# Axe--/Visual-Question-Answering

Measured on AMD Instinct MI355X. Metric: QA-pairs/sec (train step, attention model, K=1000), higher is better.
Workload: dtype f32

## Files before the change

include/coattn.h:

```cpp
#ifndef COATTN_H
#define COATTN_H

#include <stddef.h>
#include <stdint.h>

#ifdef __cplusplus
extern "C" {
#endif

#define COATTN_F32 0
#define COATTN_BF16 1

#define COATTN_IMPL_AUTO 0
#define COATTN_IMPL_GENERAL 1
#define COATTN_IMPL_FUSED 2
#define COATTN_FLAG_BF16_PROJ 4
#define COATTN_FLAG_BF16_IN 8
#define COATTN_FLAG_EXACT3 16
#define COATTN_FLAG_SPLIT2 32
#define COATTN_FLAG_F16PAIR 64
#define COATTN_FLAG_FAST16 128
#define COATTN_FLAG_BILINEAR 256
typedef struct coattn_params {
  const void* W_v; const void* b_v;
// ... 178 lines not shown
int coattn_bn_exact_geometry(int B, int H, int W, int C, int dtype, int* out);
size_t coattn_bn_exact_workspace_bytes(int B, int H, int W, int C);
int coattn_bn_exact_forward(const void* x, const void* gamma, const void* beta, void* running_mean, void* running_var,
                            double momentum, double eps, void* y, void* save_mean, void* save_invstd, void* ws, int B, int H,
                            int W, int C, int pool, int relu, int dtype, void* stream);

int coattn_conv1_bn_exact_supported(int B, int H, int W, int Cin, int Cout, int pool, int dtype);
size_t coattn_conv1_bn_exact_workspace_bytes(int B, int H, int W, int with_x);
int coattn_conv1_bn_exact_forward(const void* image, const void* weight, const void* gamma, const void* beta, void* running_mean,
                                  void* running_var, double momentum, double eps, void* x_out, void* y, void* save_mean,
                                  void* save_invstd, void* ws, int B, int H, int W, int Cin, int Cout, int pool, int dtype,
                                  void* stream);
int coattn_conv1_probe(const void* image, const void* weight, void* x, void* ws, int B, int H, int W, int order, int step,
                       int halves, int skip, void* stream);

typedef struct coattn_lstm_params      { const void *w_ih, *w_hh, *b_ih, *b_hh; } coattn_lstm_params;
typedef struct coattn_lstm_param_grads { void *w_ih, *w_hh, *b_ih, *b_hh; } coattn_lstm_param_grads;
int coattn_lstm_supported(int B, int T, int E, int H, int dtype);
int coattn_lstm_workspace_bytes(int B, int T, int E, int H, int dtype, size_t* saved, size_t* ws_fwd, size_t* ws_bwd);
int coattn_lstm_forward(const void* X, const int32_t* len, const coattn_lstm_params* p, void* out, void* x_masked,
                        void* saved, void* ws, int B, int T, int E, int H, int dtype, int flags, void* stream);
int coattn_lstm_backward(const void* X, const int32_t* len, const coattn_lstm_params* p, const void* out, const void* saved,
                         const void* g_out, const void* g_xmasked, void* dX, const coattn_lstm_param_grads* pg,
                         int accumulate, void* ws, int B, int T, int E, int H, int dtype, int flags, void* stream);

#define COATTN_IDS_I32 0
#define COATTN_IDS_I64 1
#define COATTN_EMBEDDING_CHUNK 32
int coattn_embedding_supported(long long n, long long V, int E, int dtype);
int coattn_embedding_workspace_bytes(long long n, long long V, int E, int dtype, size_t* ws_bwd);
// ... 70 lines not shown
```

visual-question-answering_amd/_lib.py:

```python
from __future__ import annotations

import ctypes as C
import os
import subprocess

_HERE = os.path.dirname(os.path.abspath(__file__))
LIB_PATH = os.environ.get("COATTN_LIB_PATH") or os.path.join(_HERE, "libcoattn_hip.so")
CSRC = os.path.join(_HERE, "csrc")

EXPORTS = ("coattn_version", "coattn_last_error", "coattn_fused_supported", "coattn_workspace_bytes",
           "coattn_forward", "coattn_attention_forward", "coattn_backward", "coattn_gemm_f32", "coattn_gemm_bf16",
           "coattn_phrase_workspace_bytes", "coattn_phrase_forward", "coattn_phrase_backward",
           "coattn_ce_workspace_bytes", "coattn_ce_forward", "coattn_linear_workspace_bytes", "coattn_linear_forward",
           "coattn_linear_wgrad_workspace_bytes", "coattn_linear_weight_grad",
           "coattn_head_workspace_bytes", "coattn_head_forward", "coattn_head_backward", "coattn_head_status",
           "coattn_ce_status", "coattn_p2p_enable_peer", "coattn_p2p_reduce_scatter", "coattn_p2p_all_gather",
           "coattn_profile_begin", "coattn_profile_end", "coattn_features_native", "coattn_status",
           "coattn_phrase_status", "coattn_status_accumulate", "coattn_phrase_status_accumulate", "coattn_infer",
           "coattn_forward_len", "coattn_infer_len", "coattn_attention_forward_len", "coattn_backward_len",
           "coattn_forward_maps", "coattn_forward_maps_len", "coattn_backward_maps", "coattn_backward_maps_len",
           "coattn_alt_workspace_bytes", "coattn_alt_forward", "coattn_alt_backward",
           "coattn_soft_loss_forward", "coattn_vqa_score", "coattn_head_forward_soft",
           "coattn_adam_workspace_bytes", "coattn_adam_step",
           "coattn_bn_supported", "coattn_bn_workspace_bytes", "coattn_bn_relu_pool_forward", "coattn_relu_pool_forward",
           "coattn_bn_exact_geometry", "coattn_bn_exact_workspace_bytes", "coattn_bn_exact_forward",
           "coattn_conv1_bn_exact_supported", "coattn_conv1_bn_exact_workspace_bytes", "coattn_conv1_bn_exact_forward",
           "coattn_conv1_probe",
           "coattn_lstm_supported", "coattn_lstm_workspace_bytes", "coattn_lstm_forward", "coattn_lstm_backward",
           "coattn_embedding_supported", "coattn_embedding_workspace_bytes", "coattn_embedding_forward",
           "coattn_embedding_backward",
           "coattn_dropout_supported", "coattn_dropout_forward", "coattn_dropout_backward",
           "coattn_features_gather_supported", "coattn_features_gather",
           "coattn_overlay_supported", "coattn_overlay_render")

F32 = 0
IDS_I32, IDS_I64 = 0, 1
BF16 = 1
IMPL_AUTO, IMPL_GENERAL, IMPL_FUSED = 0, 1, 2
FLAG_BF16_PROJ = 4
FLAG_BF16_IN = 8
FLAG_EXACT3 = 16
FLAG_SPLIT2 = 32
# ... 123 lines not shown
                                  + _int("accumulate dtype flags") + _void("stream")),
}
DROPOUT_SIGNATURES = {
    "coattn_dropout_forward": (_void("x0 y0 x1 y1") + _i64("n") + _of(C.c_float)("p") + _void("state") + _int("advance")
                               + _void("stream")),
    "coattn_dropout_backward": _void("g dx") + _i64("n") + _of(C.c_float)("p") + _void("state stream"),
}
FEATURES_SIGNATURES = {
    "coattn_features_gather": (_void("table") + _int("table_dtype") + _void("idx") + _int("idx_dtype") + _void("out bad_idx")
                               + _i64("S B") + _int("N d flags") + _void("stream")),
}
OVERLAY_SIGNATURES = {
    "coattn_overlay_render": (_void("image") + _i64("sB sC sH sW") + _void("a_v a_q q_len") + (("p", C.POINTER(OverlayParams)),)
                              + _void("out bad_maps") + _int("B L H W Gh Gw T strip_h mode") + _void("stream")),
}
_TABLE = {**SIGNATURES, **EMBEDDING_SIGNATURES, **DROPOUT_SIGNATURES, **FEATURES_SIGNATURES, **OVERLAY_SIGNATURES}
_INDEX = {name: {n: i for i, (n, _) in enumerate(sig)} for name, sig in _TABLE.items()}
_DEFAULTS = dict.fromkeys("q_len av_out aq_out saved g_av g_aq dV labels loss g_loss g_logits dv dq bad_ids bad_idx x1 y1 bad_maps".split())
_DEFAULTS.update(dv_sB=0, dv_sN=0, dv_sD=0)


def ptr(t):
    return C.c_void_p(t.data_ptr()) if t is not None else C.c_void_p(0)


def ptr_array(tensors):
    return (C.c_void_p * len(tensors))(*[t.data_ptr() for t in tensors])


def rows(t):
    step = t.stride(0) * t.element_size()
# ... 126 lines not shown
    lib.coattn_bn_workspace_bytes.restype = C.c_size_t
    lib.coattn_bn_relu_pool_forward.argtypes = ([C.c_void_p] * 6 + [C.c_double] * 2 + [C.c_void_p] * 3 + [C.c_int] * 7
                                                + [C.c_void_p])
    lib.coattn_relu_pool_forward.argtypes = [C.c_void_p] * 2 + [C.c_int] * 5 + [C.c_void_p]
    lib.coattn_bn_exact_geometry.argtypes = [C.c_int] * 5 + [C.POINTER(C.c_int)]
    lib.coattn_bn_exact_workspace_bytes.argtypes = [C.c_int] * 4
    lib.coattn_bn_exact_workspace_bytes.restype = C.c_size_t
    lib.coattn_bn_exact_forward.argtypes = ([C.c_void_p] * 5 + [C.c_double] * 2 + [C.c_void_p] * 4 + [C.c_int] * 7
                                            + [C.c_void_p])
    lib.coattn_conv1_bn_exact_supported.argtypes = [C.c_int] * 7
    lib.coattn_conv1_bn_exact_workspace_bytes.argtypes = [C.c_int] * 4
    lib.coattn_conv1_bn_exact_workspace_bytes.restype = C.c_size_t
    lib.coattn_conv1_bn_exact_forward.argtypes = ([C.c_void_p] * 6 + [C.c_double] * 2 + [C.c_void_p] * 5 + [C.c_int] * 7
                                                  + [C.c_void_p])
    lib.coattn_conv1_probe.argtypes = [C.c_void_p] * 4 + [C.c_int] * 7 + [C.c_void_p]
    lib.coattn_lstm_supported.argtypes = [C.c_int] * 5
    lib.coattn_lstm_workspace_bytes.argtypes = [C.c_int] * 5 + [C.POINTER(C.c_size_t)] * 3
    lib.coattn_lstm_forward.argtypes = ([C.c_void_p] * 2 + [C.POINTER(LstmParams)] + [C.c_void_p] * 4 + [C.c_int] * 6
                                        + [C.c_void_p])
    lib.coattn_lstm_backward.argtypes = ([C.c_void_p] * 2 + [C.POINTER(LstmParams)] + [C.c_void_p] * 5
                                         + [C.POINTER(LstmParamGrads)] + [C.c_int] + [C.c_void_p] + [C.c_int] * 6
                                         + [C.c_void_p])
    lib.coattn_embedding_supported.argtypes = [C.c_int64, C.c_int64, C.c_int, C.c_int]
    lib.coattn_embedding_workspace_bytes.argtypes = [C.c_int64, C.c_int64, C.c_int, C.c_int, C.POINTER(C.c_size_t)]
    lib.coattn_dropout_supported.argtypes = [C.c_int64]
    lib.coattn_features_gather_supported.argtypes = [C.c_int64, C.c_int64, C.c_int, C.c_int, C.c_int, C.c_int]
    lib.coattn_overlay_supported.argtypes = [C.c_int] * 9
    _lib = lib
    return lib

# ... 137 lines not shown
```

visual-question-answering_amd/csrc/api.hip:

```cpp
#include "common.h"
#include "fused.h"

#include <string.h>

static thread_local char g_err[512] = "";

void coattn_set_error(const char* fmt, ...) {
  va_list ap;
  va_start(ap, fmt);
  vsnprintf(g_err, sizeof(g_err), fmt, ap);
  va_end(ap);
}

extern "C" int coattn_version(void) { return 2100; }

namespace {
constexpr int kProfMax = 48;
struct Prof {
  bool on = false;
  int n = 0, created = 0;
  hipEvent_t ev[kProfMax + 1];
  const char* name[kProfMax];
};
thread_local Prof g_prof;
}

void prof_mark(hipStream_t s, const char* name) {
  Prof& p = g_prof;
  if (!p.on || p.n >= kProfMax) return;
// ... 837 lines not shown
```

visual-question-answering_amd/csrc/encoder.hip:

```cpp
#include <math.h>

#include "common.h"

namespace {

constexpr int kThreads = 256;
constexpr int kMaxStatBlocks = 2048;
constexpr int kPixelsPerStatBlock = 400;
constexpr int kMaxNormBlocks = 4096;
constexpr int kStatLoads = 8;

typedef double f64x2 __attribute__((ext_vector_type(2)));

inline int stat_blocks(int64_t pixels) {
  const int64_t g = pixels / kPixelsPerStatBlock;
  return g < 1 ? 1 : g > kMaxStatBlocks ? kMaxStatBlocks : (int)g;
}

inline size_t partial_bytes(int G, int C) { return (size_t)G * C * sizeof(f64x2); }

__global__ __launch_bounds__(kThreads) void bn_stats_partial_kernel(const f32x4* __restrict__ x, f64x2* __restrict__ partial,
                                                                    int64_t total4, int c4) {
  __shared__ double sh[8][kThreads];
  const int tid = threadIdx.x;
// ... 181 lines not shown
  }
  running_mean[xg] = nm;
  running_var[xg] = nv;
  save_mean[xg] = mean;
  save_invstd[xg] = invstd;
}

constexpr int kConv1Terms = 32;
constexpr int kConv1Mfmas = kConv1Terms / 2;
constexpr int kConv1Pixels = 32;

template <int D>
__device__ __forceinline__ constexpr int conv1_term(int i, int g) { return (i / D) * 2 * D + g * D + i % D; }

template <int D>
__global__ __launch_bounds__(128) void conv1_stats_miopen_kernel(
    const float* __restrict__ image, const float* __restrict__ weight, float* __restrict__ x, float* __restrict__ partial, int B,
    int H, int W, int g1, int ngrps) {
  __shared__ float lds[kConv1Pixels * 64 * 2];
  const int hh = threadIdx.x >> 6, lane = threadIdx.x & 63, g = lane >> 5, p = lane & 31;
  const int HW = H * W;
  const int pbase = blockIdx.x * kConv1Pixels, pix = pbase + p;
  const bool live = pix < HW;
  const bool full = pbase + kConv1Pixels <= HW;
  const int h = pix / W, w = pix - h * W;
  const int ch = 32 * hh + p;
  float wt[kConv1Mfmas];
  int off[kConv1Mfmas];
  unsigned real = 0;
#pragma unroll
  for (int i = 0; i < kConv1Mfmas; ++i) {
    const int k = conv1_term<D>(i, g);
    const int tap = k / 3, c = k - 3 * tap, ky = tap / 3, kx = tap - 3 * ky;
    const int ih = h + ky - 1, iw = w + kx - 1;
    const bool in = live && k < 27 && ih >= 0 && ih < H && iw >= 0 && iw < W;
    off[i] = in ? (ih * W + iw) * 3 + c : 0;
    real |= in ? 1u << i : 0u;
    const float wk = weight[ch * 27 + (k < 27 ? k : 26)];
    wt[i] = k < 27 ? wk : 0.f;
  }
  const int64_t sample = (int64_t)HW * 3;
  float even[kConv1Mfmas], odd[kConv1Mfmas];
  const float* image1 = image + (B > 1 ? sample : 0);
#pragma unroll
  for (int i = 0; i < kConv1Mfmas; ++i) even[i] = image[off[i]];
#pragma unroll
  for (int i = 0; i < kConv1Mfmas; ++i) odd[i] = image1[off[i]];
  float sum[16], sq[16];
#pragma unroll
  for (int v = 0; v < 16; ++v) sum[v] = sq[v] = 0.f;
  float* xo = x + ((int64_t)(pbase + 4 * g) * 64 + ch);
  const int64_t xstep = (int64_t)HW * 64;
  auto one_sample = [&](float (&terms)[kConv1Mfmas], int n) {
    const float* ahead = image + (int64_t)(n + 2 < B ? n + 2 : B - 1) * sample;
    f32x16 acc;
#pragma unroll
    for (int e = 0; e < 16; ++e) acc[e] = 0.f;
#pragma unroll
    for (int i = 0; i < kConv1Mfmas; ++i) {
      const float t = (real >> i) & 1u ? terms[i] : 0.f;
      acc = __builtin_amdgcn_mfma_f32_32x32x2f32(t, wt[i], acc, 0, 0, 0);
      terms[i] = ahead[off[i]];
    }
    if (full) {
#pragma unroll
      for (int v = 0; v < 16; ++v) {
        xo[(8 * (v >> 2) + (v & 3)) * 64] = acc[v];
        sum[v] += acc[v];
        sq[v] = __builtin_fmaf(acc[v], acc[v], sq[v]);
      }
    } else {
#pragma unroll
      for (int v = 0; v < 16; ++v)
        if (pbase + 8 * (v >> 2) + 4 * g + (v & 3) < HW) {
          xo[(8 * (v >> 2) + (v & 3)) * 64] = acc[v];
          sum[v] += acc[v];
          sq[v] = __builtin_fmaf(acc[v], acc[v], sq[v]);
        }
    }
    xo += xstep;
  };
  for (int n = 0; n < B; n += 2) {
    one_sample(even, n);
    if (n + 1 < B) one_sample(odd, n + 1);
  }
#pragma unroll
  for (int v = 0; v < 16; ++v) {
    const int o = ((8 * (v >> 2) + 4 * g + (v & 3)) * 64 + ch) * 2;
    lds[o] = sum[v];
    lds[o + 1] = sq[v];
  }
  __syncthreads();
  for (int red = g1 >> 1; red > 0; red >>= 1) {
#pragma unroll
    for (int v = 0; v < 16; ++v) {
// ... 62 lines not shown
    if (step == 0) {
      sacc = __builtin_fmaf(a, v, sacc);
    } else {
      const float prod = __fmul_rn(a, v);
      sacc = __fadd_rn(prod, sacc);
    }
  }
  x[i] = halves == 2 ? __fadd_rn(acc[0], acc[1]) : acc[0];
}

struct Affine {
  float mean[4], lo[4], scale[4], beta[4], gamma[4];
};

template <bool STOCK>
__device__ __forceinline__ f32x4 affine(const f32x4 v, const Affine& a) {
  f32x4 t;
#pragma unroll
  for (int e = 0; e < 4; ++e)
    t[e] = STOCK ? __builtin_fmaf(a.gamma[e], (v[e] - a.mean[e]) * a.scale[e], a.beta[e])
                 : fmaf((v[e] - a.mean[e]) - a.lo[e], a.scale[e], a.beta[e]);
  return t;
}
__device__ __forceinline__ f32x4 max_nan(const f32x4 a, const f32x4 b) {
  f32x4 m;
#pragma unroll
  for (int e = 0; e < 4; ++e) m[e] = (a[e] > b[e] || a[e] != a[e]) ? a[e] : b[e];
  return m;
}
__device__ __forceinline__ f32x4 relu_nan(const f32x4 a) {
  f32x4 r;
#pragma unroll
  for (int e = 0; e < 4; ++e) r[e] = a[e] < 0.f ? 0.f : a[e];
  return r;
}

template <bool POOL, bool AFFINE = true, bool STOCK = false>
__global__ __launch_bounds__(kThreads) void bn_relu_pool_kernel(const f32x4* __restrict__ x, const float* __restrict__ ws_f,
                                                                const float* __restrict__ scale, const float* __restrict__ gamma,
                                                                const float* __restrict__ beta, f32x4* __restrict__ y,
                                                                int H, int W, int C, int c4_shift, int64_t total4, int relu) {
  const int tid = threadIdx.x;
  const int c4 = C >> 2;
  const int cg = tid & (c4 - 1);
  Affine a;
#pragma unroll
  for (int e = 0; e < 4; ++e) {
    a.mean[e] = AFFINE ? ws_f[4 * cg + e] : 0.f;
// ... 29 lines not shown
      const int64_t ou = o + u * stride;
      live[u] = ou < total4;
      if (live[u]) {
        const uint32_t pix = (uint32_t)(ou >> c4_shift);
        const uint32_t wo = pix % Wo, r = pix / Wo, ho = r % Ho, b = r / Ho;
        const int64_t in4 = (((int64_t)b * H + 2 * ho) * W + 2 * wo) * c4 + cg;
        v[u][0] = x[in4];
        v[u][1] = x[in4 + c4];
        v[u][2] = x[in4 + row4];
        v[u][3] = x[in4 + row4 + c4];
      }
    }
#pragma unroll
    for (int u = 0; u < 2; ++u)
      if (live[u]) {
        const f32x4 t = AFFINE ? max_nan(max_nan(affine<STOCK>(v[u][0], a), affine<STOCK>(v[u][1], a)),
                                         max_nan(affine<STOCK>(v[u][2], a), affine<STOCK>(v[u][3], a)))
                               : max_nan(max_nan(v[u][0], v[u][1]), max_nan(v[u][2], v[u][3]));
        y[o + u * stride] = relu ? relu_nan(t) : t;
      }
  }
}

inline int log2_exact(int v) {
  int s = 0;
  while ((1 << s) < v) ++s;
  return s;
}

}

extern "C" int coattn_bn_supported(int B, int H, int W, int C, int pool, int dtype) {
  if (dtype != COATTN_F32 || B < 1 || H < 1 || W < 1) return 0;
  if (C < 16 || C > 512 || (C & (C - 1)) != 0) return 0;
  const int64_t limit = (int64_t)1 << 31;
// ... 183 lines not shown
                 relu, s))
    return -1;
  prof_mark(s, "bn_exact");
  return 0;
}

namespace {

constexpr int kConv1PairDistance = 8;

inline size_t conv1_partial_bytes(const BnGeom& g) { return (exact_partial_bytes(g, 64) + 255) & ~(size_t)255; }

void launch_conv1(int dist, const void* image, const void* weight, void* x, void* partial, const BnGeom& g, int B, int H, int W,
                  hipStream_t s) {
  const int blocks = (H * W + kConv1Pixels - 1) / kConv1Pixels;
  if (dist == 8)
    hipLaunchKernelGGL(conv1_stats_miopen_kernel<8>, dim3(blocks), dim3(128), 0, s, (const float*)image, (const float*)weight,
                       (float*)x, (float*)partial, B, H, W, g.g1, g.ngrps);
  else
    hipLaunchKernelGGL(conv1_stats_miopen_kernel<4>, dim3(blocks), dim3(128), 0, s, (const float*)image, (const float*)weight,
                       (float*)x, (float*)partial, B, H, W, g.g1, g.ngrps);
}

}

extern "C" int coattn_conv1_bn_exact_supported(int B, int H, int W, int Cin, int Cout, int pool, int dtype) {
  BnGeom g;
  if (Cin != 3 || Cout != 64) return 0;
  return bn_exact_geometry(B, H, W, Cout, dtype, &g) && coattn_bn_supported(B, H, W, Cout, pool, dtype) ? 1 : 0;
}

// ... 27 lines not shown
               "conv1_bn_exact_forward: x_out, y, ws, the BatchNorm vectors must be 16-byte aligned, image and weight 4-byte aligned");
  CA_CHECK_ARG(momentum >= 0.0 && momentum <= 1.0, "conv1_bn_exact_forward: momentum %g outside [0, 1]", momentum);
  CA_CHECK_ARG(eps > 0.0, "conv1_bn_exact_forward: eps %g (must be > 0)", eps);
  void* x = x_out ? x_out : (void*)((char*)ws + conv1_partial_bytes(g));
  CA_CHECK_ARG(x != y && x != image && y != image, "conv1_bn_exact_forward: image, x_out and y must be three buffers");
  hipStream_t s = (hipStream_t)stream;
  launch_conv1(kConv1PairDistance, image, weight, x, ws, g, B, H, W, s);
  CA_CHECK_LAUNCH("conv1_stats_miopen");
  if (exact_tail(x, gamma, beta, running_mean, running_var, momentum, eps, y, save_mean, save_invstd, (const f32x4*)ws, g, B, H, W,
                 Cout, pool, 1, s))
    return -1;
  prof_mark(s, "conv1_bn_exact");
  return 0;
}

extern "C" int coattn_conv1_probe(const void* image, const void* weight, void* x, void* ws, int B, int H, int W, int order, int step,
                                  int halves, int skip, void* stream) {
  BnGeom g;
  CA_CHECK_ARG(B >= 1 && H >= 1 && W >= 1 && bn_exact_geometry(B, H, W, 64, COATTN_F32, &g),
               "conv1_probe: B=%d H=%d W=%d is not a covered shape (coattn_conv1_bn_exact_supported)", B, H, W);
  CA_CHECK_ARG(image && weight && x && ws && (reinterpret_cast<uintptr_t>(x) & 15) == 0 && (reinterpret_cast<uintptr_t>(ws) & 15) == 0,
               "conv1_probe: a null or misaligned image / weight / x / ws");
  CA_CHECK_ARG(order >= -2 && order <= 13 && (step == 0 || step == 1) && (halves == 1 || halves == 2) && (skip == 0 || skip == 1),
               "conv1_probe: order=%d step=%d halves=%d skip=%d", order, step, halves, skip);
  hipStream_t s = (hipStream_t)stream;
  if (order < 0) {
    launch_conv1(order == -1 ? 8 : 4, image, weight, x, ws, g, B, H, W, s);
  } else {
    const int64_t total = (int64_t)B * H * W * 64;
    hipLaunchKernelGGL(conv1_probe_kernel, dim3((unsigned)((total + 255) / 256)), dim3(256), 0, s, (const float*)image,
// ... 6 lines not shown
```

visual-question-answering_amd/encoder.py:

```python
from __future__ import annotations

import ctypes as C
import os
import warnings

import torch
import torch.nn as nn

from . import _lib


def _pair(v):
    return tuple(v) if isinstance(v, (tuple, list)) else (v, v)


def pool_is_2x2(pool: nn.MaxPool2d) -> bool:
    stride = pool.kernel_size if pool.stride is None else pool.stride
    return (_pair(pool.kernel_size) == (2, 2) and _pair(stride) == (2, 2) and _pair(pool.padding) == (0, 0)
            and _pair(pool.dilation) == (1, 1) and not pool.ceil_mode and not pool.return_indices)


def mode() -> str:
    return {"0": "stock", "1": "bn"}.get(os.environ.get("VQA_ENCODER_FUSED", ""), "pool")

# ... 86 lines not shown


def exact_geometry(B: int, H: int, W: int, Ch: int):
    out = (C.c_int * len(GEOMETRY_FIELDS))()
    n = _lib.load().coattn_bn_exact_geometry(B, H, W, Ch, _lib.F32, out)
    return dict(zip(GEOMETRY_FIELDS, out)) if n == len(GEOMETRY_FIELDS) else None


def exact_output_fusable(z: torch.Tensor, bn: nn.BatchNorm2d, pool: bool) -> bool:
    if not output_fusable(z, bn, pool) or exact_geometry(z.shape[0], z.shape[2], z.shape[3], z.shape[1]) is None:
        return False
    return all(t.data_ptr() % 16 == 0 for t in (z, bn.weight, bn.bias, bn.running_mean, bn.running_var))


def exact_report() -> dict:
    return {k: {n: dict(t) if n == "conv1" else t for n, t in v.items()} for k, v in _exact.items()}


def _bn_exact_raw(x, weight, bias, running_mean, running_var, momentum, eps, pool: bool):
    lib = _lib.load()
    B, Ch, H, W = x.shape
    Ho, Wo = (H // 2, W // 2) if pool else (H, W)
    y = torch.empty((B, Ch, Ho, Wo), device=x.device, dtype=torch.float32, memory_format=torch.channels_last)
    save = torch.empty((2, Ch), device=x.device, dtype=torch.float32)
    ws = torch.empty((lib.coattn_bn_exact_workspace_bytes(B, H, W, Ch) + 3) // 4, device=x.device, dtype=torch.float32)
    with torch.no_grad(), _lib.on_device(x.device):
        rc = lib.coattn_bn_exact_forward(_lib.ptr(x), _lib.ptr(weight), _lib.ptr(bias), _lib.ptr(running_mean),
                                         _lib.ptr(running_var), float(momentum), float(eps), _lib.ptr(y), _lib.ptr(save[0]),
                                         _lib.ptr(save[1]), _lib.ptr(ws), B, H, W, Ch, int(pool), 1, _lib.F32,
                                         C.c_void_p(_lib.stream_ptr(x.device)))
        _lib.check(rc, "coattn_bn_exact_forward")
    return y, save[0], save[1]


def bn_exact(x: torch.Tensor, bn: nn.BatchNorm2d, pool: bool = False, conv=None) -> torch.Tensor:
    if conv is not None:
        if not conv1_inputs_fusable(x, conv, bn, pool):
            raise ValueError("bn_exact: with conv it needs a CUDA fp32 channels_last [B,3,H,W] image, a 3 -> 64 channel 3x3 / stride 1 "
                             "/ padding 1 convolution with channels_last weights and a shape coattn_conv1_bn_exact_supported "
                             "covers, got %s %s strides %s" % (tuple(x.shape), x.dtype, x.stride()))
        _, y, _, _ = _conv1_raw(x, conv.weight, bn.weight, bn.bias, bn.running_mean, bn.running_var, bn.momentum, bn.eps, pool, False)
    else:
        if not exact_output_fusable(x, bn, pool):
            raise ValueError("bn_exact: needs a CUDA fp32 channels_last [B,C,H,W] tensor of a shape coattn_bn_exact_geometry "
                             "covers, got %s %s strides %s" % (tuple(x.shape), x.dtype, x.stride()))
        y, _, _ = _bn_exact_raw(x, bn.weight, bn.bias, bn.running_mean, bn.running_var, bn.momentum, bn.eps, pool)
    if bn.num_batches_tracked is not None:
        with torch.no_grad():
            bn.num_batches_tracked.add_(1)
    return y


def _stock_chain(x: torch.Tensor, bn: nn.BatchNorm2d, pool) -> torch.Tensor:
    z = bn(x)
    if pool is None:
        return torch.relu_(z)
# ... 56 lines not shown
        return False
    for t in (bn.weight, bn.bias, bn.running_mean, bn.running_var):
        if t is None or t.dtype != torch.float32 or t.device != x.device or not t.is_contiguous() or t.data_ptr() % 16 != 0:
            return False
    if bn.num_features != 64 or x.data_ptr() % 4 != 0 or w.data_ptr() % 4 != 0:
        return False
    B, _, H, W = x.shape
    return bool(_lib.load().coattn_conv1_bn_exact_supported(B, H, W, 3, 64, int(pool), _lib.F32))


def conv1_modules_fusable(conv: nn.Conv2d, bn: nn.BatchNorm2d, pool, x: torch.Tensor) -> bool:
    return (conv1_enabled() and not torch.is_autocast_enabled() and _group_fusable(conv, bn, pool, x)
            and conv1_inputs_fusable(x, conv, bn, pool is not None))


def _conv1_raw(image, weight, gamma, beta, running_mean, running_var, momentum, eps, pool: bool, want_x: bool):
    lib = _lib.load()
    B, _, H, W = image.shape
    Ho, Wo = (H // 2, W // 2) if pool else (H, W)
    dev = image.device
    y = torch.empty((B, 64, Ho, Wo), device=dev, dtype=torch.float32, memory_format=torch.channels_last)
    x = torch.empty((B, 64, H, W), device=dev, dtype=torch.float32, memory_format=torch.channels_last) if want_x else None
    save = torch.empty((2, 64), device=dev, dtype=torch.float32)
    ws = torch.empty((lib.coattn_conv1_bn_exact_workspace_bytes(B, H, W, int(not want_x)) + 3) // 4, device=dev, dtype=torch.float32)
    with torch.no_grad(), _lib.on_device(dev):
        rc = lib.coattn_conv1_bn_exact_forward(_lib.ptr(image), _lib.ptr(weight), _lib.ptr(gamma), _lib.ptr(beta),
                                               _lib.ptr(running_mean), _lib.ptr(running_var), float(momentum), float(eps),
                                               _lib.ptr(x), _lib.ptr(y), _lib.ptr(save[0]), _lib.ptr(save[1]), _lib.ptr(ws), B, H, W,
                                               3, 64, int(pool), _lib.F32, C.c_void_p(_lib.stream_ptr(dev)))
        _lib.check(rc, "coattn_conv1_bn_exact_forward")
    return x, y, save[0], save[1]


def _conv1_stock(x: torch.Tensor, conv: nn.Conv2d, bn: nn.BatchNorm2d, pool) -> torch.Tensor:
    z = torch.nn.functional.conv2d(x, conv.weight, None, conv.stride, conv.padding, conv.dilation, conv.groups)
    return _bn_or_stock(z, bn, pool) if exact_output_fusable(z, bn, pool is not None) else _stock_chain(z, bn, pool)


def _verify_conv1(x: torch.Tensor, conv: nn.Conv2d, bn: nn.BatchNorm2d, pool, key) -> torch.Tensor:
    with torch.no_grad():
        rm0, rv0 = bn.running_mean.clone(), bn.running_var.clone()
        z = torch.nn.functional.conv2d(x, conv.weight, None, conv.stride, conv.padding, conv.dilation, conv.groups)
        if not exact_output_fusable(z, bn, pool is not None):
            return _stock_chain(z, bn, pool)
        y = _bn_or_stock(z, bn, pool)
        _, save_mean, save_invstd = torch.miopen_batch_norm(z, bn.weight, bn.bias, rm0.clone(), rv0.clone(), True,
                                                            bn.momentum, bn.eps)
        mine_x, mine_y, mine_mean, mine_invstd = _conv1_raw(x, conv.weight, bn.weight, bn.bias, rm0, rv0, bn.momentum, bn.eps,
                                                            pool is not None, True)
        names = ("x", "y", "running_mean", "running_var", "save_mean", "save_invstd")
        pairs = ((mine_x, z), (mine_y, y), (rm0, bn.running_mean), (rv0, bn.running_var), (mine_mean, save_mean),
                 (mine_invstd, save_invstd))
        flags = torch.stack([_differs(a, b) for a, b in pairs]).tolist()
    first = next((n for n, f in zip(names, flags) if f), None)
    B, _, H, W = x.shape
    _exact.setdefault(key, {"verified": False, "first_difference": None, "geometry": exact_geometry(B, H, W, 64)})["conv1"] = {
        "verified": first is None, "first_difference": first}
    if first is not None:
        warnings.warn("encoder: the one-pass first convolution does not reproduce the stock kernels for B=%d H=%d W=%d pool=%d "
                      "(%s differs); this shape stays on the stock kernels" % (B, H, W, int(pool is not None), first))
    return y


def _conv1_or_stock(x: torch.Tensor, conv: nn.Conv2d, bn: nn.BatchNorm2d, pool) -> torch.Tensor:
    B, _, H, W = x.shape
    key = (x.device.index if x.device.index is not None else torch.cuda.current_device(), B, 64, H, W, pool is not None)
    state = (_exact.get(key) or {}).get("conv1")
    if state is None:
        if torch.cuda.is_current_stream_capturing():
            return _conv1_stock(x, conv, bn, pool)
        return _verify_conv1(x, conv, bn, pool, key)
    return bn_exact(x, bn, pool is not None, conv=conv) if state["verified"] else _conv1_stock(x, conv, bn, pool)


def conv1_bn_exact_or_stock(x: torch.Tensor, conv: nn.Conv2d, bn: nn.BatchNorm2d, pool) -> torch.Tensor:
    return bn_exact_or_stock(x, bn, pool, conv=conv)
```

Baseline: 7194.

## Recompute first conv in BN normalize pass instead of storing conv output

Adds a two-pass conv1+BN path. The first pass computes only the per-channel statistics without writing the 64-channel conv activation. A second kernel recomputes the 3x3 convolution with MFMA and applies the affine, ReLU and optional pooling directly. This avoids writing and re-reading the full-resolution conv output, at the cost of doing the conv arithmetic twice. The path is on by default and is checked against the stock kernels at first use, falling back to the stored-output form if the results differ.

```diff
diff --git a/include/coattn.h b/include/coattn.h
--- a/include/coattn.h
+++ b/include/coattn.h
@@ -216,6 +216,13 @@
 int coattn_conv1_probe(const void* image, const void* weight, void* x, void* ws, int B, int H, int W, int order, int step,
                        int halves, int skip, void* stream);
 
+#define COATTN_CONV1_RECOMPUTE_CHUNK 8
+size_t coattn_conv1_bn_recompute_workspace_bytes(int B, int H, int W);
+int coattn_conv1_bn_recompute_forward(const void* image, const void* weight, const void* gamma, const void* beta,
+                                      void* running_mean, void* running_var, double momentum, double eps, void* y,
+                                      void* save_mean, void* save_invstd, void* ws, int B, int H, int W, int Cin, int Cout, int pool,
+                                      int dtype, void* stream);
+
 typedef struct coattn_lstm_params      { const void *w_ih, *w_hh, *b_ih, *b_hh; } coattn_lstm_params;
 typedef struct coattn_lstm_param_grads { void *w_ih, *w_hh, *b_ih, *b_hh; } coattn_lstm_param_grads;
 int coattn_lstm_supported(int B, int T, int E, int H, int dtype);
diff --git a/visual-question-answering_amd/_lib.py b/visual-question-answering_amd/_lib.py
--- a/visual-question-answering_amd/_lib.py
+++ b/visual-question-answering_amd/_lib.py
@@ -25,7 +25,7 @@
            "coattn_bn_supported", "coattn_bn_workspace_bytes", "coattn_bn_relu_pool_forward", "coattn_relu_pool_forward",
            "coattn_bn_exact_geometry", "coattn_bn_exact_workspace_bytes", "coattn_bn_exact_forward",
            "coattn_conv1_bn_exact_supported", "coattn_conv1_bn_exact_workspace_bytes", "coattn_conv1_bn_exact_forward",
-           "coattn_conv1_probe",
+           "coattn_conv1_probe", "coattn_conv1_bn_recompute_workspace_bytes", "coattn_conv1_bn_recompute_forward",
            "coattn_lstm_supported", "coattn_lstm_workspace_bytes", "coattn_lstm_forward", "coattn_lstm_backward",
            "coattn_embedding_supported", "coattn_embedding_workspace_bytes", "coattn_embedding_forward",
            "coattn_embedding_backward",
@@ -179,7 +179,14 @@
     "coattn_overlay_render": (_void("image") + _i64("sB sC sH sW") + _void("a_v a_q q_len") + (("p", C.POINTER(OverlayParams)),)
                               + _void("out bad_maps") + _int("B L H W Gh Gw T strip_h mode") + _void("stream")),
 }
-_TABLE = {**SIGNATURES, **EMBEDDING_SIGNATURES, **DROPOUT_SIGNATURES, **FEATURES_SIGNATURES, **OVERLAY_SIGNATURES}
+CONV1_RECOMPUTE_CHUNK = 8
+CONV1_SIGNATURES = {
+    "coattn_conv1_bn_recompute_forward": (_void("image weight gamma beta running_mean running_var") + _of(C.c_double)("momentum eps")
+                                          + _void("y save_mean save_invstd ws") + _int("B H W Cin Cout pool dtype")
+                                          + _void("stream")),
+}
+_TABLE = {**SIGNATURES, **EMBEDDING_SIGNATURES, **DROPOUT_SIGNATURES, **FEATURES_SIGNATURES, **OVERLAY_SIGNATURES,
+          **CONV1_SIGNATURES}
 _INDEX = {name: {n: i for i, (n, _) in enumerate(sig)} for name, sig in _TABLE.items()}
 _DEFAULTS = dict.fromkeys("q_len av_out aq_out saved g_av g_aq dV labels loss g_loss g_logits dv dq bad_ids bad_idx x1 y1 bad_maps".split())
 _DEFAULTS.update(dv_sB=0, dv_sN=0, dv_sD=0)
@@ -336,6 +343,8 @@
     lib.coattn_conv1_bn_exact_forward.argtypes = ([C.c_void_p] * 6 + [C.c_double] * 2 + [C.c_void_p] * 5 + [C.c_int] * 7
                                                   + [C.c_void_p])
     lib.coattn_conv1_probe.argtypes = [C.c_void_p] * 4 + [C.c_int] * 7 + [C.c_void_p]
+    lib.coattn_conv1_bn_recompute_workspace_bytes.argtypes = [C.c_int] * 3
+    lib.coattn_conv1_bn_recompute_workspace_bytes.restype = C.c_size_t
     lib.coattn_lstm_supported.argtypes = [C.c_int] * 5
     lib.coattn_lstm_workspace_bytes.argtypes = [C.c_int] * 5 + [C.POINTER(C.c_size_t)] * 3
     lib.coattn_lstm_forward.argtypes = ([C.c_void_p] * 2 + [C.POINTER(LstmParams)] + [C.c_void_p] * 4 + [C.c_int] * 6
diff --git a/visual-question-answering_amd/csrc/api.hip b/visual-question-answering_amd/csrc/api.hip
--- a/visual-question-answering_amd/csrc/api.hip
+++ b/visual-question-answering_amd/csrc/api.hip
@@ -12,7 +12,7 @@
   va_end(ap);
 }
 
-extern "C" int coattn_version(void) { return 2100; }
+extern "C" int coattn_version(void) { return 2200; }
 
 namespace {
 constexpr int kProfMax = 48;
diff --git a/visual-question-answering_amd/csrc/encoder.hip b/visual-question-answering_amd/csrc/encoder.hip
--- a/visual-question-answering_amd/csrc/encoder.hip
+++ b/visual-question-answering_amd/csrc/encoder.hip
@@ -1,4 +1,6 @@
 #include <math.h>
+
+#include <type_traits>
 
 #include "common.h"
 
@@ -219,7 +221,60 @@
 __device__ __forceinline__ constexpr int conv1_term(int i, int g) { return (i / D) * 2 * D + g * D + i % D; }
 
 template <int D>
-__global__ __launch_bounds__(128) void conv1_stats_miopen_kernel(
+__device__ __forceinline__ unsigned conv1_operands(const float* __restrict__ weight, int ch, int g, int h, int w, bool live, int H,
+                                                   int W, float (&wt)[kConv1Mfmas], int (&off)[kConv1Mfmas]) {
+  unsigned real = 0;
+#pragma unroll
+  for (int i = 0; i < kConv1Mfmas; ++i) {
+    const int k = conv1_term<D>(i, g);
+    const int tap = k / 3, c = k - 3 * tap, ky = tap / 3, kx = tap - 3 * ky;
+    const int ih = h + ky - 1, iw = w + kx - 1;
+    const bool in = live && k < 27 && ih >= 0 && ih < H && iw >= 0 && iw < W;
+    off[i] = in ? (ih * W + iw) * 3 + c : 0;
+    real |= in ? 1u << i : 0u;
+    const float wk = weight[ch * 27 + (k < 27 ? k : 26)];
+    wt[i] = k < 27 ? wk : 0.f;
+  }
+  return real;
+}
+
+__device__ __forceinline__ float conv1_load(const float* __restrict__ base, int off) { return base[off]; }
+__device__ __forceinline__ float conv1_load(const float* __restrict__ base, unsigned boff) {
+  return *reinterpret_cast<const float*>(reinterpret_cast<const char*>(base) + boff);
+}
+
+template <typename Off>
+__device__ __forceinline__ f32x16 conv1_chain(float (&terms)[kConv1Mfmas], const float (&wt)[kConv1Mfmas],
+                                              const Off (&off)[kConv1Mfmas], unsigned real, const float* __restrict__ ahead) {
+  f32x16 acc;
+#pragma unroll
+  for (int e = 0; e < 16; ++e) acc[e] = 0.f;
+#pragma unroll
+  for (int i = 0; i < kConv1Mfmas; ++i) {
+    const float t = (real >> i) & 1u ? terms[i] : 0.f;
+    acc = __builtin_amdgcn_mfma_f32_32x32x2f32(t, wt[i], acc, 0, 0, 0);
+    terms[i] = conv1_load(ahead, off[i]);
+  }
+  return acc;
+}
+
+template <typename Off>
+__device__ __forceinline__ void conv1_chain2(float (&terms)[kConv1Mfmas], const float (&wt0)[kConv1Mfmas],
+                                             const float (&wt1)[kConv1Mfmas], const Off (&off)[kConv1Mfmas], unsigned real,
+                                             const float* __restrict__ ahead, f32x16& acc0, f32x16& acc1) {
+#pragma unroll
+  for (int e = 0; e < 16; ++e) acc0[e] = acc1[e] = 0.f;
+#pragma unroll
+  for (int i = 0; i < kConv1Mfmas; ++i) {
+    const float t = (real >> i) & 1u ? terms[i] : 0.f;
+    acc0 = __builtin_amdgcn_mfma_f32_32x32x2f32(t, wt0[i], acc0, 0, 0, 0);
+    acc1 = __builtin_amdgcn_mfma_f32_32x32x2f32(t, wt1[i], acc1, 0, 0, 0);
+    terms[i] = conv1_load(ahead, off[i]);
+  }
+}
+
+template <int D, bool STORE = true>
+__global__ __launch_bounds__(128) __attribute__((amdgpu_waves_per_eu(STORE ? 1 : 3))) void conv1_stats_miopen_kernel(
     const float* __restrict__ image, const float* __restrict__ weight, float* __restrict__ x, float* __restrict__ partial, int B,
     int H, int W, int g1, int ngrps) {
   __shared__ float lds[kConv1Pixels * 64 * 2];
@@ -232,45 +287,29 @@
   const int ch = 32 * hh + p;
   float wt[kConv1Mfmas];
   int off[kConv1Mfmas];
-  unsigned real = 0;
-#pragma unroll
-  for (int i = 0; i < kConv1Mfmas; ++i) {
-    const int k = conv1_term<D>(i, g);
-    const int tap = k / 3, c = k - 3 * tap, ky = tap / 3, kx = tap - 3 * ky;
-    const int ih = h + ky - 1, iw = w + kx - 1;
-    const bool in = live && k < 27 && ih >= 0 && ih < H && iw >= 0 && iw < W;
-    off[i] = in ? (ih * W + iw) * 3 + c : 0;
-    real |= in ? 1u << i : 0u;
-    const float wk = weight[ch * 27 + (k < 27 ? k : 26)];
-    wt[i] = k < 27 ? wk : 0.f;
-  }
+  const unsigned real = conv1_operands<D>(weight, ch, g, h, w, live, H, W, wt, off);
+  typename std::conditional<STORE, int, unsigned>::type toff[kConv1Mfmas];
+#pragma unroll
+  for (int i = 0; i < kConv1Mfmas; ++i) toff[i] = STORE ? off[i] : (unsigned)off[i] * 4u;
   const int64_t sample = (int64_t)HW * 3;
   float even[kConv1Mfmas], odd[kConv1Mfmas];
   const float* image1 = image + (B > 1 ? sample : 0);
 #pragma unroll
-  for (int i = 0; i < kConv1Mfmas; ++i) even[i] = image[off[i]];
-#pragma unroll
-  for (int i = 0; i < kConv1Mfmas; ++i) odd[i] = image1[off[i]];
+  for (int i = 0; i < kConv1Mfmas; ++i) even[i] = conv1_load(image, toff[i]);
+#pragma unroll
+  for (int i = 0; i < kConv1Mfmas; ++i) odd[i] = conv1_load(image1, toff[i]);
   float sum[16], sq[16];
 #pragma unroll
   for (int v = 0; v < 16; ++v) sum[v] = sq[v] = 0.f;
-  float* xo = x + ((int64_t)(pbase + 4 * g) * 64 + ch);
+  float* xo = STORE ? x + ((int64_t)(pbase + 4 * g) * 64 + ch) : nullptr;
   const int64_t xstep = (int64_t)HW * 64;
   auto one_sample = [&](float (&terms)[kConv1Mfmas], int n) {
     const float* ahead = image + (int64_t)(n + 2 < B ? n + 2 : B - 1) * sample;
-    f32x16 acc;
-#pragma unroll
-    for (int e = 0; e < 16; ++e) acc[e] = 0.f;
-#pragma unroll
-    for (int i = 0; i < kConv1Mfmas; ++i) {
-      const float t = (real >> i) & 1u ? terms[i] : 0.f;
-      acc = __builtin_amdgcn_mfma_f32_32x32x2f32(t, wt[i], acc, 0, 0, 0);
-      terms[i] = ahead[off[i]];
-    }
+    const f32x16 acc = conv1_chain(terms, wt, toff, real, ahead);
     if (full) {
 #pragma unroll
       for (int v = 0; v < 16; ++v) {
-        xo[(8 * (v >> 2) + (v & 3)) * 64] = acc[v];
+        if constexpr (STORE) xo[(8 * (v >> 2) + (v & 3)) * 64] = acc[v];
         sum[v] += acc[v];
         sq[v] = __builtin_fmaf(acc[v], acc[v], sq[v]);
       }
@@ -278,12 +317,12 @@
 #pragma unroll
       for (int v = 0; v < 16; ++v)
         if (pbase + 8 * (v >> 2) + 4 * g + (v & 3) < HW) {
-          xo[(8 * (v >> 2) + (v & 3)) * 64] = acc[v];
+          if constexpr (STORE) xo[(8 * (v >> 2) + (v & 3)) * 64] = acc[v];
           sum[v] += acc[v];
           sq[v] = __builtin_fmaf(acc[v], acc[v], sq[v]);
         }
     }
-    xo += xstep;
+    if constexpr (STORE) xo += xstep;
   };
   for (int n = 0; n < B; n += 2) {
     one_sample(even, n);
@@ -376,24 +415,32 @@
 };
 
 template <bool STOCK>
+__device__ __forceinline__ float affine1(float v, float mean, float lo, float scale, float gamma, float beta) {
+  return STOCK ? __builtin_fmaf(gamma, (v - mean) * scale, beta) : fmaf((v - mean) - lo, scale, beta);
+}
+__device__ __forceinline__ float max_nan1(float a, float b) { return (a > b || a != a) ? a : b; }
+__device__ __forceinline__ float relu_nan1(float a) { return a < 0.f ? 0.f : a; }
+__device__ __forceinline__ float window_max1(float t00, float t01, float t10, float t11) {
+  return max_nan1(max_nan1(t00, t01), max_nan1(t10, t11));
+}
+
+template <bool STOCK>
 __device__ __forceinline__ f32x4 affine(const f32x4 v, const Affine& a) {
   f32x4 t;
 #pragma unroll
-  for (int e = 0; e < 4; ++e)
-    t[e] = STOCK ? __builtin_fmaf(a.gamma[e], (v[e] - a.mean[e]) * a.scale[e], a.beta[e])
-                 : fmaf((v[e] - a.mean[e]) - a.lo[e], a.scale[e], a.beta[e]);
+  for (int e = 0; e < 4; ++e) t[e] = affine1<STOCK>(v[e], a.mean[e], a.lo[e], a.scale[e], a.gamma[e], a.beta[e]);
   return t;
 }
-__device__ __forceinline__ f32x4 max_nan(const f32x4 a, const f32x4 b) {
+__device__ __forceinline__ f32x4 window_max(const f32x4 t00, const f32x4 t01, const f32x4 t10, const f32x4 t11) {
   f32x4 m;
 #pragma unroll
-  for (int e = 0; e < 4; ++e) m[e] = (a[e] > b[e] || a[e] != a[e]) ? a[e] : b[e];
+  for (int e = 0; e < 4; ++e) m[e] = window_max1(t00[e], t01[e], t10[e], t11[e]);
   return m;
 }
 __device__ __forceinline__ f32x4 relu_nan(const f32x4 a) {
   f32x4 r;
 #pragma unroll
-  for (int e = 0; e < 4; ++e) r[e] = a[e] < 0.f ? 0.f : a[e];
+  for (int e = 0; e < 4; ++e) r[e] = relu_nan1(a[e]);
   return r;
 }
 
@@ -453,11 +500,79 @@
 #pragma unroll
     for (int u = 0; u < 2; ++u)
       if (live[u]) {
-        const f32x4 t = AFFINE ? max_nan(max_nan(affine<STOCK>(v[u][0], a), affine<STOCK>(v[u][1], a)),
-                                         max_nan(affine<STOCK>(v[u][2], a), affine<STOCK>(v[u][3], a)))
-                               : max_nan(max_nan(v[u][0], v[u][1]), max_nan(v[u][2], v[u][3]));
+        const f32x4 t = AFFINE ? window_max(affine<STOCK>(v[u][0], a), affine<STOCK>(v[u][1], a), affine<STOCK>(v[u][2], a),
+                                            affine<STOCK>(v[u][3], a))
+                               : window_max(v[u][0], v[u][1], v[u][2], v[u][3]);
         y[o + u * stride] = relu ? relu_nan(t) : t;
       }
+  }
+}
+
+constexpr int kConv1NormChunk = COATTN_CONV1_RECOMPUTE_CHUNK;
+
+template <int D, bool POOL>
+__global__ __launch_bounds__(64) __attribute__((amdgpu_waves_per_eu(3))) void conv1_norm_pool_kernel(
+    const float* __restrict__ image, const float* __restrict__ weight, const float* __restrict__ save_mean,
+    const float* __restrict__ save_invstd, const float* __restrict__ gamma, const float* __restrict__ beta, float* __restrict__ y,
+    int B, int H, int W, int cbs) {
+  const int lane = threadIdx.x, g = lane >> 5, p = lane & 31;
+  const int HW = H * W, Ho = H >> 1, Wo = W >> 1;
+  const int n0 = blockIdx.y * kConv1NormChunk, n1 = n0 + kConv1NormChunk < B ? n0 + kConv1NormChunk : B;
+  const int ho = POOL ? blockIdx.x / cbs : 0, cb = POOL ? blockIdx.x - ho * cbs : 0;
+  const int pbase = blockIdx.x * kConv1Pixels;
+  const int pix = pbase + p;
+  const bool live = POOL ? 8 * cb + (p >> 2) < Wo : pix < HW;
+  const int h = POOL ? 2 * ho + ((p >> 1) & 1) : pix / W;
+  const int w = POOL ? 2 * (8 * cb + (p >> 2)) + (p & 1) : pix - h * W;
+  float wt0[kConv1Mfmas], wt1[kConv1Mfmas];
+  int off[kConv1Mfmas];
+  const unsigned real = conv1_operands<D>(weight, p, g, h, w, live, H, W, wt0, off);
+  conv1_operands<D>(weight, 32 + p, g, h, w, live, H, W, wt1, off);
+  unsigned boff[kConv1Mfmas];
+#pragma unroll
+  for (int i = 0; i < kConv1Mfmas; ++i) boff[i] = (unsigned)off[i] * 4u;
+  const float mean[2] = {save_mean[p], save_mean[32 + p]}, invstd[2] = {save_invstd[p], save_invstd[32 + p]};
+  const float gm[2] = {gamma[p], gamma[32 + p]}, bt[2] = {beta[p], beta[32 + p]};
+  const int64_t sample = (int64_t)HW * 3;
+  float even[kConv1Mfmas], odd[kConv1Mfmas];
+  const float* image0 = image + (int64_t)n0 * sample;
+  const float* image1 = image + (int64_t)(n0 + 1 < n1 ? n0 + 1 : n0) * sample;
+#pragma unroll
+  for (int i = 0; i < kConv1Mfmas; ++i) even[i] = conv1_load(image0, boff[i]);
+#pragma unroll
+  for (int i = 0; i < kConv1Mfmas; ++i) odd[i] = conv1_load(image1, boff[i]);
+  const int wo = 8 * cb + g;
+  float* yo = POOL ? y + ((((int64_t)n0 * Ho + ho) * Wo + wo) * 64 + p) : y + (((int64_t)n0 * HW + pbase + 4 * g) * 64 + p);
+  const int64_t ystep = POOL ? (int64_t)Ho * Wo * 64 : (int64_t)HW * 64;
+  const bool full = POOL ? 8 * cb + 8 <= Wo : pbase + kConv1Pixels <= HW;
+  auto one_sample = [&](float (&terms)[kConv1Mfmas], int n) {
+    const float* ahead = image + (int64_t)(n + 2 < n1 ? n + 2 : n1 - 1) * sample;
+    f32x16 acc[2];
+    conv1_chain2(terms, wt0, wt1, boff, real, ahead, acc[0], acc[1]);
+#pragma unroll
+    for (int hh = 0; hh < 2; ++hh) {
+      if (POOL) {
+#pragma unroll
+        for (int b = 0; b < 4; ++b) {
+          const float m = window_max1(affine1<true>(acc[hh][4 * b], mean[hh], 0.f, invstd[hh], gm[hh], bt[hh]),
+                                      affine1<true>(acc[hh][4 * b + 1], mean[hh], 0.f, invstd[hh], gm[hh], bt[hh]),
+                                      affine1<true>(acc[hh][4 * b + 2], mean[hh], 0.f, invstd[hh], gm[hh], bt[hh]),
+                                      affine1<true>(acc[hh][4 * b + 3], mean[hh], 0.f, invstd[hh], gm[hh], bt[hh]));
+          if (full || wo + 2 * b < Wo) yo[2 * b * 64 + 32 * hh] = relu_nan1(m);
+        }
+      } else {
+#pragma unroll
+        for (int v = 0; v < 16; ++v)
+          if (full || pbase + 8 * (v >> 2) + 4 * g + (v & 3) < HW)
+            yo[(8 * (v >> 2) + (v & 3)) * 64 + 32 * hh] =
+                relu_nan1(affine1<true>(acc[hh][v], mean[hh], 0.f, invstd[hh], gm[hh], bt[hh]));
+      }
+    }
+    yo += ystep;
+  };
+  for (int n = n0; n < n1; n += 2) {
+    one_sample(even, n);
+    if (n + 1 < n1) one_sample(odd, n + 1);
   }
 }
 
@@ -671,7 +786,10 @@
 void launch_conv1(int dist, const void* image, const void* weight, void* x, void* partial, const BnGeom& g, int B, int H, int W,
                   hipStream_t s) {
   const int blocks = (H * W + kConv1Pixels - 1) / kConv1Pixels;
-  if (dist == 8)
+  if (!x)
+    hipLaunchKernelGGL((conv1_stats_miopen_kernel<kConv1PairDistance, false>), dim3(blocks), dim3(128), 0, s, (const float*)image,
+                       (const float*)weight, (float*)nullptr, (float*)partial, B, H, W, g.g1, g.ngrps);
+  else if (dist == 8)
     hipLaunchKernelGGL(conv1_stats_miopen_kernel<8>, dim3(blocks), dim3(128), 0, s, (const float*)image, (const float*)weight,
                        (float*)x, (float*)partial, B, H, W, g.g1, g.ngrps);
   else
@@ -729,6 +847,66 @@
   return 0;
 }
 
+extern "C" size_t coattn_conv1_bn_recompute_workspace_bytes(int B, int H, int W) {
+  BnGeom g;
+  if (!bn_exact_geometry(B, H, W, 64, COATTN_F32, &g)) {
+    coattn_set_error("conv1_bn_recompute_workspace_bytes: B=%d H=%d W=%d is not a covered shape (coattn_conv1_bn_exact_supported)", B, H, W);
+    return 0;
+  }
+  return conv1_partial_bytes(g);
+}
+
+extern "C" int coattn_conv1_bn_recompute_forward(const void* image, const void* weight, const void* gamma, const void* beta,
+                                                 void* running_mean, void* running_var, double momentum, double eps, void* y,
+                                                 void* save_mean, void* save_invstd, void* ws, int B, int H, int W, int Cin,
+                                                 int Cout, int pool, int dtype, void* stream) {
+  CA_CHECK_ARG(B >= 1 && H >= 1 && W >= 1 && Cin >= 1 && Cout >= 1, "conv1_bn_recompute_forward: B=%d H=%d W=%d Cin=%d Cout=%d (all must be >= 1)",
+               B, H, W, Cin, Cout);
+  BnGeom g;
+  CA_CHECK_ARG(coattn_conv1_bn_exact_supported(B, H, W, Cin, Cout, pool, dtype) && bn_exact_geometry(B, H, W, Cout, dtype, &g),
+               "conv1_bn_recompute_forward: B=%d H=%d W=%d Cin=%d Cout=%d pool=%d dtype=%d is not a covered shape "
+               "(coattn_conv1_bn_exact_supported)", B, H, W, Cin, Cout, pool, dtype);
+  CA_CHECK_ARG(image && weight && gamma && beta && running_mean && running_var && y && save_mean && save_invstd && ws,
+               "conv1_bn_recompute_forward: a null image / weight / gamma / beta / running_mean / running_var / y / save_mean / "
+               "save_invstd / ws");
+  CA_CHECK_ARG(((reinterpret_cast<uintptr_t>(y) | reinterpret_cast<uintptr_t>(ws) | reinterpret_cast<uintptr_t>(gamma) |
+                 reinterpret_cast<uintptr_t>(beta) | reinterpret_cast<uintptr_t>(running_mean) |
+                 reinterpret_cast<uintptr_t>(running_var) | reinterpret_cast<uintptr_t>(save_mean) |
+                 reinterpret_cast<uintptr_t>(save_invstd)) & 15) == 0 &&
+                   ((reinterpret_cast<uintptr_t>(image) | reinterpret_cast<uintptr_t>(weight)) & 3) == 0,
+               "conv1_bn_recompute_forward: y, ws, the BatchNorm vectors must be 16-byte aligned, image and weight 4-byte aligned");
+  CA_CHECK_ARG(momentum >= 0.0 && momentum <= 1.0, "conv1_bn_recompute_forward: momentum %g outside [0, 1]", momentum);
+  CA_CHECK_ARG(eps > 0.0, "conv1_bn_recompute_forward: eps %g (must be > 0)", eps);
+  CA_CHECK_ARG(y != image, "conv1_bn_recompute_forward: image and y must be two buffers");
+  hipStream_t s = (hipStream_t)stream;
+  launch_conv1(kConv1PairDistance, image, weight, nullptr, ws, g, B, H, W, s);
+  CA_CHECK_LAUNCH("conv1_stats_miopen");
+  prof_mark(s, "conv1_stats");
+  const int64_t pixels = (int64_t)B * H * W;
+  const float n_f = (float)pixels;
+  const float inhw = (float)(1.0 / (double)pixels), unbias = pixels == 1 ? 1.f : n_f / (n_f - 1.f);
+  const int c4 = Cout / 4;
+  hipLaunchKernelGGL(bn_finalize_miopen_kernel, dim3(c4 / g.f0), dim3(g.f0, g.f1, g.f2),
+                     (size_t)2 * g.f0 * g.f1 * g.f2 * sizeof(f32x4), s, (const f32x4*)ws, g, c4, inhw, unbias, (float)momentum,
+                     (float)eps, (f32x4*)running_mean, (f32x4*)running_var, (f32x4*)save_mean, (f32x4*)save_invstd);
+  CA_CHECK_LAUNCH("bn_finalize_miopen");
+  prof_mark(s, "conv1_finalize");
+  const int chunks = (B + kConv1NormChunk - 1) / kConv1NormChunk;
+  if (pool) {
+    const int cbs = (W / 2 + 7) / 8;
+    hipLaunchKernelGGL((conv1_norm_pool_kernel<kConv1PairDistance, true>), dim3((unsigned)((H / 2) * cbs), chunks), dim3(64), 0, s,
+                       (const float*)image, (const float*)weight, (const float*)save_mean, (const float*)save_invstd,
+                       (const float*)gamma, (const float*)beta, (float*)y, B, H, W, cbs);
+  } else {
+    hipLaunchKernelGGL((conv1_norm_pool_kernel<kConv1PairDistance, false>), dim3((H * W + kConv1Pixels - 1) / kConv1Pixels, chunks),
+                       dim3(64), 0, s, (const float*)image, (const float*)weight, (const float*)save_mean,
+                       (const float*)save_invstd, (const float*)gamma, (const float*)beta, (float*)y, B, H, W, 0);
+  }
+  CA_CHECK_LAUNCH("conv1_norm_pool");
+  prof_mark(s, "conv1_norm_pool");
+  return 0;
+}
+
 extern "C" int coattn_conv1_probe(const void* image, const void* weight, void* x, void* ws, int B, int H, int W, int order, int step,
                                   int halves, int skip, void* stream) {
   BnGeom g;
diff --git a/visual-question-answering_amd/encoder.py b/visual-question-answering_amd/encoder.py
--- a/visual-question-answering_amd/encoder.py
+++ b/visual-question-answering_amd/encoder.py
@@ -124,7 +124,7 @@
 
 
 def exact_report() -> dict:
-    return {k: {n: dict(t) if n == "conv1" else t for n, t in v.items()} for k, v in _exact.items()}
+    return {k: {n: dict(t) if n in ("conv1", "conv1_recompute") else t for n, t in v.items()} for k, v in _exact.items()}
 
 
 def _bn_exact_raw(x, weight, bias, running_mean, running_var, momentum, eps, pool: bool):
@@ -143,13 +143,14 @@
     return y, save[0], save[1]
 
 
-def bn_exact(x: torch.Tensor, bn: nn.BatchNorm2d, pool: bool = False, conv=None) -> torch.Tensor:
+def bn_exact(x: torch.Tensor, bn: nn.BatchNorm2d, pool: bool = False, conv=None, recompute=None) -> torch.Tensor:
     if conv is not None:
         if not conv1_inputs_fusable(x, conv, bn, pool):
             raise ValueError("bn_exact: with conv it needs a CUDA fp32 channels_last [B,3,H,W] image, a 3 -> 64 channel 3x3 / stride 1 "
                              "/ padding 1 convolution with channels_last weights and a shape coattn_conv1_bn_exact_supported "
                              "covers, got %s %s strides %s" % (tuple(x.shape), x.dtype, x.stride()))
-        _, y, _, _ = _conv1_raw(x, conv.weight, bn.weight, bn.bias, bn.running_mean, bn.running_var, bn.momentum, bn.eps, pool, False)
+        _, y, _, _ = _conv1_raw(x, conv.weight, bn.weight, bn.bias, bn.running_mean, bn.running_var, bn.momentum, bn.eps, pool, False,
+                                recompute)
     else:
         if not exact_output_fusable(x, bn, pool):
             raise ValueError("bn_exact: needs a CUDA fp32 channels_last [B,C,H,W] tensor of a shape coattn_bn_exact_geometry "
@@ -236,7 +237,29 @@
             and conv1_inputs_fusable(x, conv, bn, pool is not None))
 
 
-def _conv1_raw(image, weight, gamma, beta, running_mean, running_var, momentum, eps, pool: bool, want_x: bool):
+def conv1_recompute_enabled() -> bool:
+    return os.environ.get("VQA_ENCODER_CONV1_RECOMPUTE", "1") != "0"
+
+
+def _conv1_recompute_raw(image, weight, gamma, beta, running_mean, running_var, momentum, eps, pool: bool):
+    lib = _lib.load()
+    B, _, H, W = image.shape
+    Ho, Wo = (H // 2, W // 2) if pool else (H, W)
+    dev = image.device
+    y = torch.empty((B, 64, Ho, Wo), device=dev, dtype=torch.float32, memory_format=torch.channels_last)
+    save = torch.empty((2, 64), device=dev, dtype=torch.float32)
+    ws = torch.empty((lib.coattn_conv1_bn_recompute_workspace_bytes(B, H, W) + 3) // 4, device=dev, dtype=torch.float32)
+    with torch.no_grad(), _lib.on_device(dev):
+        _lib.bind("coattn_conv1_bn_recompute_forward", image=image, weight=weight, gamma=gamma, beta=beta,
+                  running_mean=running_mean, running_var=running_var, momentum=float(momentum), eps=float(eps), y=y,
+                  save_mean=save[0], save_invstd=save[1], ws=ws, B=B, H=H, W=W, Cin=3, Cout=64, pool=int(pool), dtype=_lib.F32,
+                  stream=_lib.stream_ptr(dev))()
+    return y, save[0], save[1]
+
+
+def _conv1_raw(image, weight, gamma, beta, running_mean, running_var, momentum, eps, pool: bool, want_x: bool, recompute=None):
+    if not want_x and (conv1_recompute_enabled() if recompute is None else recompute):
+        return (None,) + _conv1_recompute_raw(image, weight, gamma, beta, running_mean, running_var, momentum, eps, pool)
     lib = _lib.load()
     B, _, H, W = image.shape
     Ho, Wo = (H // 2, W // 2) if pool else (H, W)
@@ -262,6 +285,7 @@
 def _verify_conv1(x: torch.Tensor, conv: nn.Conv2d, bn: nn.BatchNorm2d, pool, key) -> torch.Tensor:
     with torch.no_grad():
         rm0, rv0 = bn.running_mean.clone(), bn.running_var.clone()
+        rm1, rv1 = rm0.clone(), rv0.clone()
         z = torch.nn.functional.conv2d(x, conv.weight, None, conv.stride, conv.padding, conv.dilation, conv.groups)
         if not exact_output_fusable(z, bn, pool is not None):
             return _stock_chain(z, bn, pool)
@@ -274,13 +298,29 @@
         pairs = ((mine_x, z), (mine_y, y), (rm0, bn.running_mean), (rv0, bn.running_var), (mine_mean, save_mean),
                  (mine_invstd, save_invstd))
         flags = torch.stack([_differs(a, b) for a, b in pairs]).tolist()
-    first = next((n for n, f in zip(names, flags) if f), None)
+        first = next((n for n, f in zip(names, flags) if f), None)
+        del mine_x
+        again = None
+        if first is None and conv1_recompute_enabled():
+            re_y, re_mean, re_invstd = _conv1_recompute_raw(x, conv.weight, bn.weight, bn.bias, rm1, rv1, bn.momentum, bn.eps,
+                                                            pool is not None)
+            pairs = ((re_y, y), (rm1, bn.running_mean), (rv1, bn.running_var), (re_mean, save_mean), (re_invstd, save_invstd))
+            flags = torch.stack([_differs(a, b) for a, b in pairs]).tolist()
+            again = next((n for n, f in zip(names[1:], flags) if f), None)
     B, _, H, W = x.shape
-    _exact.setdefault(key, {"verified": False, "first_difference": None, "geometry": exact_geometry(B, H, W, 64)})["conv1"] = {
-        "verified": first is None, "first_difference": first}
+    entry = _exact.setdefault(key, {"verified": False, "first_difference": None, "geometry": exact_geometry(B, H, W, 64)})
+    entry["conv1"] = {"verified": first is None, "first_difference": first}
+    if first is None and conv1_recompute_enabled():
+        entry["conv1_recompute"] = {"verified": again is None, "first_difference": again}
+    else:
+        entry.pop("conv1_recompute", None)
     if first is not None:
         warnings.warn("encoder: the one-pass first convolution does not reproduce the stock kernels for B=%d H=%d W=%d pool=%d "
                       "(%s differs); this shape stays on the stock kernels" % (B, H, W, int(pool is not None), first))
+    elif again is not None:
+        warnings.warn("encoder: the recomputed first convolution does not reproduce the stock kernels for B=%d H=%d W=%d pool=%d "
+                      "(%s differs); this shape keeps the form that stores the convolution output"
+                      % (B, H, W, int(pool is not None), again))
     return y
 
 
@@ -292,7 +332,18 @@
         if torch.cuda.is_current_stream_capturing():
             return _conv1_stock(x, conv, bn, pool)
         return _verify_conv1(x, conv, bn, pool, key)
-    return bn_exact(x, bn, pool is not None, conv=conv) if state["verified"] else _conv1_stock(x, conv, bn, pool)
+    if not state["verified"]:
+        return _conv1_stock(x, conv, bn, pool)
+    recompute = conv1_recompute_enabled()
+    if recompute:
+        again = _exact[key].get("conv1_recompute")
+        if again is None:
+            if not torch.cuda.is_current_stream_capturing():
+                return _verify_conv1(x, conv, bn, pool, key)
+            recompute = False
+        else:
+            recompute = again["verified"]
+    return bn_exact(x, bn, pool is not None, conv=conv, recompute=recompute)
 
 
 def conv1_bn_exact_or_stock(x: torch.Tensor, conv: nn.Conv2d, bn: nn.BatchNorm2d, pool) -> torch.Tensor:
```

Measured after the change: 7349, median of 6. +2.1%, better.
